# lgalke/aae-recommender

Measured on NVIDIA B200. Metric: AAE train item-sets/sec, higher is better.
Workload: dtype f32

## Files before the change

aae-recommender_b200/csrc/dec_out_tc.cu:

```cuda
#include "common.cuh"

#ifndef TC_WAIT_HINT
#define TC_WAIT_HINT 0x989680u
#endif
#ifndef TC_WAIT_SLEEP_NS
#define TC_WAIT_SLEEP_NS 40
#endif
#ifndef TC2_CW
#define TC2_CW 16
#endif
#ifndef TC2_G1_FIRST
#define TC2_G1_FIRST 1
#endif

namespace aae {
AAE_DEFINE_TRACE_SETTER(trace_set_tc)
namespace tc {

constexpr int TN = 32;
constexpr int BM = 128;
constexpr int NT = 512;
constexpr int CW = 8;
constexpr int CORE = 128;

__device__ __forceinline__ uint32_t smem_u32(const void* p) { return (uint32_t)__cvta_generic_to_shared(p); }

__device__ __forceinline__ uint64_t make_desc(uint32_t saddr, uint32_t lbo_bytes, uint32_t sbo_bytes) {
  uint64_t d = 0;
  d |= (uint64_t)((saddr >> 4) & 0x3FFFu);
  d |= (uint64_t)((lbo_bytes >> 4) & 0x3FFFu) << 16;
  d |= (uint64_t)((sbo_bytes >> 4) & 0x3FFFu) << 32;
  d |= (uint64_t)1 << 46;
  return d;
}
__device__ __forceinline__ uint64_t make_desc_sw(uint32_t saddr, uint32_t lbo_bytes, uint32_t sbo_bytes, uint32_t layout_type) {
  return make_desc(saddr, lbo_bytes, sbo_bytes) | ((uint64_t)layout_type << 61);
}
__host__ __device__ constexpr uint32_t make_idesc(int M, int N, int a_mn_major, int b_mn_major) {
  return (1u << 4) | (2u << 7) | (2u << 10) | ((uint32_t)a_mn_major << 15) | ((uint32_t)b_mn_major << 16) |
         ((uint32_t)(N >> 3) << 17) | ((uint32_t)(M >> 4) << 24);
}
__device__ __forceinline__ void mma_tf32(uint32_t d_tmem, uint64_t adesc, uint64_t bdesc, uint32_t idesc,
                                         uint32_t accumulate) {
  asm volatile(
      "{\n\t"
      ".reg .pred p;\n\t"
      "setp.ne.b32 p, %4, 0;\n\t"
      "tcgen05.mma.cta_group::1.kind::tf32 [%0], %1, %2, %3, p;\n\t"
      "}\n" ::"r"(d_tmem), "l"(adesc), "l"(bdesc), "r"(idesc), "r"(accumulate)
      : "memory");
}
__device__ __forceinline__ void mma_tf32_ts(uint32_t d_tmem, uint32_t a_tmem, uint64_t bdesc, uint32_t idesc,
                                            uint32_t accumulate) {
  asm volatile(
      "{\n\t"
      ".reg .pred p;\n\t"
      "setp.ne.b32 p, %4, 0;\n\t"
      "tcgen05.mma.cta_group::1.kind::tf32 [%0], [%1], %2, %3, p;\n\t"
      "}\n" ::"r"(d_tmem), "r"(a_tmem), "l"(bdesc), "r"(idesc), "r"(accumulate)
      : "memory");
}
__device__ __forceinline__ void mma_commit(uint64_t* bar) {
  asm volatile("tcgen05.commit.cta_group::1.mbarrier::arrive::one.shared::cluster.b64 [%0];" ::"r"(smem_u32(bar))
               : "memory");
}
__device__ __forceinline__ void mbar_init(uint64_t* bar, uint32_t count) {
  asm volatile("mbarrier.init.shared::cta.b64 [%0], %1;" ::"r"(smem_u32(bar)), "r"(count) : "memory");
}
__device__ __forceinline__ void mbar_wait(uint64_t* bar, uint32_t parity) {
  uint32_t done = 0;
  uint32_t spins = 0;
  while (!done) {
    if (spins) __nanosleep(TC_WAIT_SLEEP_NS);
    if (++spins > (1u << 22)) __trap();
    asm volatile(
        "{\n\t"
        ".reg .pred p;\n\t"
        "mbarrier.try_wait.parity.shared::cta.b64 p, [%1], %2, %3;\n\t"
        "selp.u32 %0, 1, 0, p;\n\t"
        "}\n"
        : "=r"(done)
        : "r"(smem_u32(bar)), "r"(parity), "r"(TC_WAIT_HINT)
        : "memory");
  }
}
__device__ __forceinline__ bool elect_one() {
  uint32_t pred;
  asm volatile(
      "{\n\t"
      ".reg .pred p;\n\t"
      "elect.sync _|p, 0xffffffff;\n\t"
      "selp.u32 %0, 1, 0, p;\n\t"
      "}\n"
      : "=r"(pred));
  return pred != 0;
}
__device__ __forceinline__ void fence_async_smem() { asm volatile("fence.proxy.async.shared::cta;" ::: "memory"); }
__device__ __forceinline__ void tc_fence_before() { asm volatile("tcgen05.fence::before_thread_sync;" ::: "memory"); }
__device__ __forceinline__ void tc_fence_after() { asm volatile("tcgen05.fence::after_thread_sync;" ::: "memory"); }

__device__ __forceinline__ void tmem_alloc(uint32_t* dst_smem, uint32_t ncols) {
  asm volatile("tcgen05.alloc.cta_group::1.sync.aligned.shared::cta.b32 [%0], %1;" ::"r"(smem_u32(dst_smem)),
               "r"(ncols)
               : "memory");
  asm volatile("tcgen05.relinquish_alloc_permit.cta_group::1.sync.aligned;" ::: "memory");
}
__device__ __forceinline__ void tmem_dealloc(uint32_t taddr, uint32_t ncols) {
  asm volatile("tcgen05.dealloc.cta_group::1.sync.aligned.b32 %0, %1;" ::"r"(taddr), "r"(ncols) : "memory");
}
__device__ __forceinline__ void tmem_ld16(uint32_t taddr, float* v) {
  uint32_t r[16];
  asm volatile(
      "tcgen05.ld.sync.aligned.32x32b.x16.b32 {%0,%1,%2,%3,%4,%5,%6,%7,%8,%9,%10,%11,%12,%13,%14,%15}, [%16];"
      : "=r"(r[0]), "=r"(r[1]), "=r"(r[2]), "=r"(r[3]), "=r"(r[4]), "=r"(r[5]), "=r"(r[6]), "=r"(r[7]), "=r"(r[8]),
        "=r"(r[9]), "=r"(r[10]), "=r"(r[11]), "=r"(r[12]), "=r"(r[13]), "=r"(r[14]), "=r"(r[15])
      : "r"(taddr)
      : "memory");
  asm volatile("tcgen05.wait::ld.sync.aligned;" ::: "memory");
#pragma unroll
  for (int i = 0; i < 16; ++i) v[i] = __uint_as_float(r[i]);
}

__device__ __forceinline__ void tmem_st16(uint32_t taddr, const float* v) {
  asm volatile(
      "tcgen05.st.sync.aligned.32x32b.x16.b32 [%0], {%1,%2,%3,%4,%5,%6,%7,%8,%9,%10,%11,%12,%13,%14,%15,%16};" ::"r"(taddr),
      "r"(__float_as_uint(v[0])), "r"(__float_as_uint(v[1])), "r"(__float_as_uint(v[2])), "r"(__float_as_uint(v[3])),
      "r"(__float_as_uint(v[4])), "r"(__float_as_uint(v[5])), "r"(__float_as_uint(v[6])), "r"(__float_as_uint(v[7])),
      "r"(__float_as_uint(v[8])), "r"(__float_as_uint(v[9])), "r"(__float_as_uint(v[10])), "r"(__float_as_uint(v[11])),
      "r"(__float_as_uint(v[12])), "r"(__float_as_uint(v[13])), "r"(__float_as_uint(v[14])), "r"(__float_as_uint(v[15]))
      : "memory");
}
__device__ __forceinline__ void tmem_st_wait() { asm volatile("tcgen05.wait::st.sync.aligned;" ::: "memory"); }

__device__ __forceinline__ void tmem_ld8(uint32_t taddr, float* v) {
  uint32_t r[8];
  asm volatile("tcgen05.ld.sync.aligned.32x32b.x8.b32 {%0,%1,%2,%3,%4,%5,%6,%7}, [%8];"
               : "=r"(r[0]), "=r"(r[1]), "=r"(r[2]), "=r"(r[3]), "=r"(r[4]), "=r"(r[5]), "=r"(r[6]), "=r"(r[7])
               : "r"(taddr)
               : "memory");
  asm volatile("tcgen05.wait::ld.sync.aligned;" ::: "memory");
#pragma unroll
  for (int i = 0; i < 8; ++i) v[i] = __uint_as_float(r[i]);
}
__device__ __forceinline__ void tmem_ld8_issue(uint32_t taddr, uint32_t* r) {
  asm volatile("tcgen05.ld.sync.aligned.32x32b.x8.b32 {%0,%1,%2,%3,%4,%5,%6,%7}, [%8];"
               : "=r"(r[0]), "=r"(r[1]), "=r"(r[2]), "=r"(r[3]), "=r"(r[4]), "=r"(r[5]), "=r"(r[6]), "=r"(r[7])
               : "r"(taddr)
               : "memory");
}
__device__ __forceinline__ void tmem_ld8_wait(uint32_t* r, float* v) {
  asm volatile("tcgen05.wait::ld.sync.aligned;"
               : "+r"(r[0]), "+r"(r[1]), "+r"(r[2]), "+r"(r[3]), "+r"(r[4]), "+r"(r[5]), "+r"(r[6]), "+r"(r[7])::"memory");
#pragma unroll
  for (int i = 0; i < 8; ++i) v[i] = __uint_as_float(r[i]);
}
__device__ __forceinline__ void tmem_st8(uint32_t taddr, const float* v) {
  asm volatile("tcgen05.st.sync.aligned.32x32b.x8.b32 [%0], {%1,%2,%3,%4,%5,%6,%7,%8};" ::"r"(taddr),
               "r"(__float_as_uint(v[0])), "r"(__float_as_uint(v[1])), "r"(__float_as_uint(v[2])),
               "r"(__float_as_uint(v[3])), "r"(__float_as_uint(v[4])), "r"(__float_as_uint(v[5])),
               "r"(__float_as_uint(v[6])), "r"(__float_as_uint(v[7]))
               : "memory");
}
template <int N> struct TmemIO;
template <> struct TmemIO<8> {
  static __device__ __forceinline__ void ld_issue(uint32_t taddr, uint32_t* r) {
    asm volatile("tcgen05.ld.sync.aligned.32x32b.x8.b32 {%0,%1,%2,%3,%4,%5,%6,%7}, [%8];"
                 : "=r"(r[0]), "=r"(r[1]), "=r"(r[2]), "=r"(r[3]), "=r"(r[4]), "=r"(r[5]), "=r"(r[6]), "=r"(r[7])
                 : "r"(taddr)
                 : "memory");
  }
  static __device__ __forceinline__ void ld_wait(uint32_t* r) {
    asm volatile("tcgen05.wait::ld.sync.aligned;"
                 : "+r"(r[0]), "+r"(r[1]), "+r"(r[2]), "+r"(r[3]), "+r"(r[4]), "+r"(r[5]), "+r"(r[6]), "+r"(r[7])::"memory");
  }
  static __device__ __forceinline__ void st(uint32_t taddr, const float* v) { tmem_st8(taddr, v); }
};
// ... 373 lines not shown
          if (k < H) {
            size_t off = (size_t)(v0 + v) * H + k;
            Wd3[off] = p; __stcs(mW + off, m); __stcs(vW + off, vv);
          } else {
            bd3[v0 + v] = p; mb[v0 + v] = m; vb[v0 + v] = vv;
          }
        }
      }
    }
    tc_fence_before();
    __syncthreads();
  }
  tc_fence_after();
  if (dh_started) {
    for (int c = cpart; c < g.Np / CW; c += NT / 128) {
      float d[CW];
      tmem_ld8(lane_addr + TM_DH + c * CW, d);
      if (brow < B) {
#pragma unroll
        for (int j = 0; j < CW; ++j) {
          int kk = c * CW + j;
          if (kk < H) atomicAdd(dh2 + (size_t)brow * H + kk, d[j]);
        }
      }
    }
  }
  float s = warp_sum(loss_local);
  if (lane == 0) red[warp] = s;
  tc_fence_before();
  __syncthreads();
  if (tid == 0) {
    double tot = 0.0;
    for (int w = 0; w < NT / 32; ++w) tot += (double)red[w];
    atomicAdd(loss_sum, tot);
  }
  if (warp == 0) tmem_dealloc(tmem, TMEM_COLS);
}

struct RowCursor2 {
  int pos, end, n0, n1, n2, n3;
};
__device__ __forceinline__ void cursor_init(RowCursor2& c, const int32_t* __restrict__ indices, int pos, int end) {
  c.pos = pos;
  c.end = end;
  c.n0 = (pos < end) ? __ldg(indices + pos) : 0x7fffffff;
  c.n1 = (pos + 1 < end) ? __ldg(indices + pos + 1) : 0x7fffffff;
  c.n2 = (pos + 2 < end) ? __ldg(indices + pos + 2) : 0x7fffffff;
  c.n3 = (pos + 3 < end) ? __ldg(indices + pos + 3) : 0x7fffffff;
}
__device__ __forceinline__ void cursor_advance(RowCursor2& c, const int32_t* __restrict__ indices) {
  c.n0 = c.n1;
  c.n1 = c.n2;
  c.n2 = c.n3;
  ++c.pos;
  c.n3 = (c.pos + 3 < c.end) ? __ldg(indices + c.pos + 3) : 0x7fffffff;
}
__device__ __forceinline__ uint32_t tile_targets2(RowCursor2& c, const int32_t* __restrict__ indices, int v0g) {
  while (c.n0 < v0g) cursor_advance(c, indices);
  uint32_t m = 0;
  while (c.n0 < v0g + TN) {
    m |= 1u << (c.n0 - v0g);
    cursor_advance(c, indices);
  }
  return m;
}
__device__ __forceinline__ void prefetch_l2_bulk(const void* p, uint32_t bytes) {
  if (bytes >= 16u)
    asm volatile("cp.async.bulk.prefetch.L2.global [%0], %1;" ::"l"(p), "r"(bytes & ~15u) : "memory");
}

constexpr uint32_t T2_Z = 0, T2_DW = 64, T2_DZH = 128, T2_DZL = 160, T2_DH = 192;

__device__ __forceinline__ void named_bar_sync(int id, int n) { asm volatile("bar.sync %0, %1;" ::"r"(id), "r"(n) : "memory"); }
__device__ __forceinline__ void named_bar_arrive(int id, int n) { asm volatile("bar.arrive %0, %1;" ::"r"(id), "r"(n) : "memory"); }

__device__ __forceinline__ float ex2_approx(float x) {
  float r;
  asm("ex2.approx.ftz.f32 %0, %1;" : "=f"(r) : "f"(x));
  return r;
}
__device__ __forceinline__ float lg2_approx(float x) {
  float r;
  asm("lg2.approx.ftz.f32 %0, %1;" : "=f"(r) : "f"(x));
  return r;
}
__device__ __forceinline__ float bce_neg_fast(float z, float inv_n, float& dz) {
  float u = ex2_approx(-1.4426950408889634f * fabsf(z));
  float t = 1.0f + u;
  float r = rcp_approx(t);
  float x = (z >= 0.f) ? r : u * r;
  dz = x * inv_n;
  return fmaf(lg2_approx(t), 0.6931471805599453f, fmaxf(z, 0.f));
}

template <int NCH, int NW>
__device__ __forceinline__ void make_wchunks_t(WChunk* wc, const Geom& g) {
  const int ncg = g.Kp / 4;
  const int r = threadIdx.x & 31, w = threadIdx.x >> 5;
#pragma unroll
  for (int j = 0; j < NCH; ++j) {
    int cg = w + NW * j;
    wc[j].goff = -2;
    if (cg < ncg) {
      int c = cg * 4;
      wc[j].goff = (c + 3 < g.H) ? r * g.H + c : (c == g.H ? -1 : -3);
    }
    wc[j].wb_off = (uint32_t)(r >> 3) * g.wb_sbo + (uint32_t)cg * CORE + (uint32_t)(r & 7) * 16u;
    wc[j].wt_off = (uint32_t)(cg >> 1) * g.wt_sbo + (uint32_t)(r >> 2) * g.wt_lbo + (uint32_t)(cg & 1) * 64u +
                   (uint32_t)(r & 3) * 4u;
  }
}
template <int NCH>
__device__ __forceinline__ void load_w_regs_t(float4* wr, const WChunk* wc, const float* __restrict__ Wd3,
                                              const float* __restrict__ bd3, int H, int v0, int nv) {
  const int r = threadIdx.x & 31;
#pragma unroll
  for (int j = 0; j < NCH; ++j) {
    float4 x = make_float4(0.f, 0.f, 0.f, 0.f);
    if (r < nv) {
      if (wc[j].goff >= 0) x = __ldcs(reinterpret_cast<const float4*>(Wd3 + (size_t)v0 * H + wc[j].goff));
      else if (wc[j].goff == -1) x.x = __ldg(bd3 + v0 + r);
    }
    wr[j] = x;
  }
}
template <int NCH>
__device__ __forceinline__ void store_wb_regs(const float4* wr, const WChunk* wc, unsigned char* wb_hi,
                                              unsigned char* wb_lo, bool with_lo) {
#pragma unroll
  for (int j = 0; j < NCH; ++j) {
    if (wc[j].goff == -2) continue;
    float4 x = wr[j];
    pin4(x);
    float4 h = make_float4(tf32_hi(x.x), tf32_hi(x.y), tf32_hi(x.z), tf32_hi(x.w));
    *reinterpret_cast<float4*>(wb_hi + wc[j].wb_off) = h;
    if (with_lo) *reinterpret_cast<float4*>(wb_lo + wc[j].wb_off) = make_float4(x.x - h.x, x.y - h.y, x.z - h.z, x.w - h.w);
  }
}
template <int NCH>
__device__ __forceinline__ void store_wt_regs(const float4* wr, const WChunk* wc, unsigned char* wt_hi,
                                              unsigned char* wt_lo, bool with_lo) {
#pragma unroll
  for (int j = 0; j < NCH; ++j) {
    if (wc[j].goff == -2) continue;
    float4 x = wr[j];
    float4 h = make_float4(tf32_hi(x.x), tf32_hi(x.y), tf32_hi(x.z), tf32_hi(x.w));
    float* th = reinterpret_cast<float*>(wt_hi + wc[j].wt_off);
    th[0] = h.x; th[4] = h.y; th[8] = h.z; th[12] = h.w;
    if (with_lo) {
      float* tl = reinterpret_cast<float*>(wt_lo + wc[j].wt_off);
      tl[0] = x.x - h.x; tl[4] = x.y - h.y; tl[8] = x.z - h.z; tl[12] = x.w - h.w;
    }
  }
}

__device__ __forceinline__ void mbar_arrive_expect_tx(uint64_t* bar, uint32_t bytes) {
  asm volatile("mbarrier.arrive.expect_tx.shared::cta.b64 _, [%0], %1;" ::"r"(smem_u32(bar)), "r"(bytes) : "memory");
}
__device__ __forceinline__ void mbar_arrive(uint64_t* bar) {
  asm volatile("mbarrier.arrive.shared::cta.b64 _, [%0];" ::"r"(smem_u32(bar)) : "memory");
}
__device__ __forceinline__ void bulk_g2s(void* dst_smem, const void* src, uint32_t bytes, uint64_t* bar) {
  asm volatile("cp.async.bulk.shared::cluster.global.mbarrier::complete_tx::bytes [%0], [%1], %2, [%3];" ::"r"(
                   smem_u32(dst_smem)),
               "l"(src), "r"(bytes), "r"(smem_u32(bar))
               : "memory");
}

#ifndef K3_PF_MV
#define K3_PF_MV 1
#endif
#ifndef K3_PF_AHEAD
#define K3_PF_AHEAD 4
#endif
#ifdef K3X_TRACE
static __device__ long long k3x_tr[32 * 16];
#define K3X_MARK(it, slot) do { if (blockIdx.x == 0 && (it) >= 8 && (it) < 40 && (threadIdx.x & 31) == 0) k3x_tr[((it) - 8) * 16 + (slot)] = clock64(); } while (0)
#else
#define K3X_MARK(it, slot) do { } while (0)
#endif
template <int CWT> struct Tc2Cfg {
  static constexpr int NPART = TN / CWT;
  static constexpr int NWE = 4 * NPART;
  static constexpr int NTT = 32 * NWE + 32;
  static constexpr int NTHR = 64 * NWE + 64;
  static constexpr int WCHT = 32 / NWE;
  static_assert(NTHR <= 1024, "two epilogue roles of 4*TN/CWT warps each: CWT = 16");
};
template <int SPLIT, int HC, int CWT, int MODE>
__global__ void __launch_bounds__(Tc2Cfg<CWT>::NTHR, 1) dec_out_train_tc2_kernel(
    const float* __restrict__ h2, int B, int Hrt, float* __restrict__ Wd3, float* __restrict__ bd3,
    float* __restrict__ mW, float* __restrict__ vW, float* __restrict__ mb, float* __restrict__ vb, int v_begin,
    int Vloc, const int32_t* __restrict__ indptr, const int32_t* __restrict__ indices, float inv_n,
    const aae_step_state* __restrict__ st, float* __restrict__ dh2, double* __restrict__ loss_sum, int smem_total,
    float* __restrict__ gW, float* __restrict__ gB) {
  constexpr bool kAdam = (MODE == 0 || MODE == 3);
  extern __shared__ __align__(1024) unsigned char smem[];
  __shared__ uint64_t bar_g1, bar_g23;
  __shared__ uint64_t bar_stage;
  __shared__ uint64_t bar_dw[2];
  __shared__ uint64_t bar_dwfree[2];
  __shared__ uint32_t tmem_base_s;
  constexpr int NPART = Tc2Cfg<CWT>::NPART, NWE = Tc2Cfg<CWT>::NWE, NTT = Tc2Cfg<CWT>::NTT, WCHT = Tc2Cfg<CWT>::WCHT;
  constexpr int NTHR = Tc2Cfg<CWT>::NTHR;
  __shared__ float red[NWE];
  const int H = HC ? HC : Hrt;
  const Geom g = make_geom(H);
  constexpr bool with_lo = (SPLIT == 3);
  const int BK = (B + 7) & ~7;
  const uint32_t hb_eff = (uint32_t)(BK / 8) * g.hb_sbo;
  unsigned char* hb_hi = smem;
  unsigned char* hb_lo = hb_hi + hb_eff;
  unsigned char* wb_hi = hb_lo + hb_eff;
  unsigned char* wb_lo = wb_hi + g.wb_bytes;
  unsigned char* wt_hi = wb_lo + g.wb_bytes;
  unsigned char* wt_lo = wt_hi + g.wt_bytes;
  unsigned char* dt_hi = wt_lo + g.wt_bytes;
  unsigned char* dt_lo = dt_hi + g.dt_bytes;
  float* sW = reinterpret_cast<float*>(dt_lo + g.dt_bytes);
  float* sM = sW + TN * H;
  float* sV = sM + TN * H;
  float* sB = sV + TN * H;
  const int tid = threadIdx.x, warp = tid >> 5, lane = tid & 31;
  const int n_tiles = (Vloc + TN - 1) / TN;
  const int G = gridDim.x;
  const int n_my = (n_tiles - (int)blockIdx.x + G - 1) / G;
  const uint32_t T2_HTH = T2_DH + (uint32_t)g.Np, T2_HTL = T2_HTH + (uint32_t)BK;

  trace_mark(TR_K3, 0);
  if (warp == 0) K3X_MARK(39, 0);
  if (warp == 2 * NWE) tmem_alloc(&tmem_base_s, TMEM_COLS);
  if (tid == 0) {
    mbar_init(&bar_g1, 1);
    mbar_init(&bar_g23, 1);
    mbar_init(&bar_stage, 1);
    mbar_init(&bar_dw[0], 1);
    mbar_init(&bar_dw[1], 1);
    mbar_init(&bar_dwfree[0], NWE);
    mbar_init(&bar_dwfree[1], NWE);
    asm volatile("fence.mbarrier_init.release.cluster;" ::: "memory");
  }
  constexpr int HB_BATCH = 5;
  const int ncg0 = g.Kp / 4;
  float4 hbx[HB_BATCH];
#pragma unroll
  for (int u = 0; u < HB_BATCH; ++u) {
    const int q = tid + u * NTHR;
    float4 x = make_float4(0.f, 0.f, 0.f, 0.f);
    if (q < BK * ncg0) {
      const int r = q / ncg0, c = (q - r * ncg0) * 4;
      if (r < B) {
        if (c + 3 < H) x = *reinterpret_cast<const float4*>(h2 + (size_t)r * H + c);
        else if (c == H) x.x = 1.0f;
      }
    }
    hbx[u] = x;
  }
  for (int q = tid; q < smem_total / 16; q += NTHR) reinterpret_cast<float4*>(smem)[q] = make_float4(0, 0, 0, 0);
  tc_fence_before();
  __syncthreads();
  tc_fence_after();
  const uint32_t tmem = tmem_base_s;
  if (warp == 0) K3X_MARK(39, 1);
  if (warp < 2 * NWE) {
    const int q4 = warp & 3, part = warp >> 2;
    const uint32_t lane_addr = tmem + ((uint32_t)(q4 * 32) << 16);
    const int k = q4 * 32 + lane;
    constexpr int NP4 = 2 * NPART;
    for (int c0 = part; c0 < BK / 8; c0 += 2 * NP4) {
      float x[16];
#pragma unroll
      for (int u = 0; u < 2; ++u) {
        const int c = c0 + u * NP4;
#pragma unroll
        for (int j = 0; j < 8; ++j) {
          const int b = c * 8 + j;
          float v = 0.f;
          if (c < BK / 8 && b < B) v = (k < H) ? h2[(size_t)b * H + k] : (k == H ? 1.0f : 0.f);
          x[u * 8 + j] = v;
        }
      }
#pragma unroll
      for (int u = 0; u < 2; ++u) {
        const int c = c0 + u * NP4;
        if (c < BK / 8) {
          float hi[8], lo[8];
#pragma unroll
          for (int j = 0; j < 8; ++j) {
            hi[j] = tf32_hi(x[u * 8 + j]);
            lo[j] = x[u * 8 + j] - hi[j];
          }
          tmem_st8(lane_addr + T2_HTH + c * 8, hi);
          if (with_lo) tmem_st8(lane_addr + T2_HTL + c * 8, lo);
        }
      }
    }
    tmem_st_wait();
  }
#pragma unroll
  for (int u = 0; u < HB_BATCH; ++u) {
    const int q = tid + u * NTHR;
    if (q < BK * ncg0) {
      const int r = q / ncg0, cg = q - r * ncg0;
      store_split4(hb_hi, hb_lo, r, cg, g.hb_sbo, hbx[u], with_lo);
    }
  }
// ... 338 lines not shown
    if (warp == 0) K3X_MARK(39, 6);
    {
      const int nch = g.Np / CWT;
      const int rot = (int)(blockIdx.x % (unsigned)nch);
      for (int c = cpart; c < nch; c += NPART) {
        int cc = c + rot;
        if (cc >= nch) cc -= nch;
        float d[CWT];
        {
          uint32_t dr[CWT];
          TmemIO<CWT>::ld_issue(lane_addr + T2_DH + cc * CWT, dr);
          TmemIO<CWT>::ld_wait(dr);
#pragma unroll
          for (int j = 0; j < CWT; ++j) d[j] = __uint_as_float(dr[j]);
        }
        if (brow < B) {
          float* dst = dh2 + (size_t)brow * H + cc * CWT;
#pragma unroll
          for (int j = 0; j < CWT; j += 4) {
            if (cc * CWT + j + 3 < H)
              asm volatile("red.global.add.v4.f32 [%0], {%1, %2, %3, %4};" ::"l"(dst + j), "f"(d[j]), "f"(d[j + 1]),
                           "f"(d[j + 2]), "f"(d[j + 3])
                           : "memory");
          }
        }
      }
    }
    float s = warp_sum(loss_local);
    if (lane == 0) red[warp] = s;
    if (warp == 0) K3X_MARK(39, 7);
  } else {
    const int we = warp - NWE;
    const int q4 = we & 3, cpart = we >> 2;
    const uint32_t lane_addr = tmem + ((uint32_t)(q4 * 32) << 16);
    const int brow = q4 * 32 + lane;
    const AdamK ak = adam_load(st, 0);
    const int kb = H & 31;
    const bool bias_warp = (q4 == (H >> 5));
    const int jb = brow - (H + 1);
    const bool is_bias = (jb >= 0 && jb < CWT);
    float* const eW = is_bias ? bd3 : Wd3;
    float* const eM = is_bias ? mb : mW;
    float* const eV = is_bias ? vb : vW;
    const float* const sWp = is_bias ? sB + cpart * CWT + jb : sW + cpart * CWT * H + brow;
    const float* const sMp = is_bias ? sB + TN + cpart * CWT + jb : sM + cpart * CWT * H + brow;
    const float* const sVp = is_bias ? sB + 2 * TN + cpart * CWT + jb : sV + cpart * CWT * H + brow;
    const int ecnt_full = is_bias ? 1 : (brow < H ? CWT : 0);
    uint32_t phase_e = 0, ph_dw0 = 0, ph_dw1 = 0;
    const uint32_t rt_zero = (uint32_t)smem_total >> 31;
    for (int jt = 0; jt < n_my; ++jt) {
      const int tile = blockIdx.x + jt * G;
      const int v0 = tile * TN;
      const int nv = min(TN, Vloc - v0);
      size_t eoff;
      int ecnt;
      if (is_bias) {
        eoff = (size_t)v0 + cpart * CWT + jb;
        ecnt = (cpart * CWT + jb < nv) ? 1 : 0;
      } else {
        eoff = (size_t)(v0 + cpart * CWT) * H + brow;
        ecnt = (brow < H) ? max(0, min(CWT, nv - cpart * CWT)) : 0;
      }
      float* pW = eW + eoff;
      float* pM = eM + eoff;
      float* pV = eV + eoff;
      float* pG = (MODE != 0) ? ((is_bias ? gB : gW) + eoff) : nullptr;
      float pw[CWT], pm[CWT], pv[CWT], pg[CWT];
#pragma unroll
      for (int j = 0; j < CWT; ++j) pw[j] = pm[j] = pv[j] = 0.f;
      if (MODE == 2 || MODE == 3) {
#pragma unroll
        for (int j = 0; j < CWT; ++j) pg[j] = (j < ecnt) ? pG[(size_t)j * H] : 0.f;
      }
      if (warp == NWE) K3X_MARK(jt, 8);
      mbar_wait(&bar_stage, phase_e);
      phase_e ^= 1;
      if (warp == NWE) K3X_MARK(jt, 9);
#ifdef K3X_NO_E2LD
      if (false) {
#else
      if (kAdam) {
#endif
        if (nv == TN) {
#pragma unroll
          for (int j = 0; j < CWT; ++j) {
            if (j < ecnt_full) {
              pw[j] = sWp[j * H];
              pm[j] = sMp[j * H];
              pv[j] = sVp[j * H];
            }
          }
        } else {
#pragma unroll
          for (int j = 0; j < CWT; ++j) {
            if (j < ecnt) {
              pw[j] = pW[(size_t)j * H];
              pm[j] = pM[(size_t)j * H];
              pv[j] = pV[(size_t)j * H];
            }
          }
        }
      }
      if (jt + 1 < n_my) {
        uint32_t dep = 0u;
#pragma unroll
        for (int j = 0; j < CWT; ++j) dep ^= __float_as_uint(pw[j]) ^ __float_as_uint(pm[j]) ^ __float_as_uint(pv[j]);
        named_bar_arrive(2 + (int)(dep & rt_zero), NTT);
      }
      if (jt & 1) { mbar_wait(&bar_dw[1], ph_dw1); ph_dw1 ^= 1; } else { mbar_wait(&bar_dw[0], ph_dw0); ph_dw0 ^= 1; }
      tc_fence_after();
      if (warp == NWE) K3X_MARK(jt, 10);
      float gw[CWT];
      {
        uint32_t gr[CWT];
        TmemIO<CWT>::ld_issue(lane_addr + T2_DW + (uint32_t)(jt & 1) * 32u + cpart * CWT, gr);
        TmemIO<CWT>::ld_wait(gr);
#pragma unroll
        for (int j = 0; j < CWT; ++j) gw[j] = __uint_as_float(gr[j]);
      }
      tc_fence_before();
      __syncwarp();
      if (lane == 0) mbar_arrive(&bar_dwfree[jt & 1]);
      if (bias_warp) {
        float gb = 0.f;
#pragma unroll
        for (int j = 0; j < CWT; ++j) {
          float t = __shfl_sync(0xffffffffu, gw[j], kb);
          if (jb == j) gb = t;
        }
        if (is_bias) gw[0] = gb;
      }
      if (MODE == 2 || MODE == 3) {
#pragma unroll
        for (int j = 0; j < CWT; ++j) gw[j] += pg[j];
      }
      if (kAdam) {
        float dn[CWT];
#ifndef K3X_NO_E2MATH
#pragma unroll
        for (int j = 0; j < CWT; ++j) pm[j] = fmaf(ak.w1, gw[j] - pm[j], pm[j]);
#pragma unroll
        for (int j = 0; j < CWT; ++j) pv[j] = fmaf(ak.w2 * gw[j], gw[j], pv[j] * ak.beta2);
#pragma unroll
        for (int j = 0; j < CWT; ++j) dn[j] = fmaf(sqrt_approx(pv[j]), ak.inv_bc2_sqrt, ak.eps);
#pragma unroll
        for (int j = 0; j < CWT; ++j) dn[j] = pm[j] * rcp_approx(dn[j]);
#pragma unroll
        for (int j = 0; j < CWT; ++j) pw[j] = fmaf(-ak.step_size, dn[j], pw[j]);
#else
#pragma unroll
        for (int j = 0; j < CWT; ++j) { dn[j] = gw[j]; pw[j] += dn[j]; }
#endif
#ifndef K3X_NO_E2ST
#pragma unroll
        for (int j = 0; j < CWT; ++j) {
          if (j < ecnt) {
            pW[(size_t)j * H] = pw[j];
            __stcs(pM + (size_t)j * H, pm[j]);
            __stcs(pV + (size_t)j * H, pv[j]);
          }
        }
#else
        if (pw[0] + pm[1] + pv[2] == 1.2345e30f) pW[0] = pw[3];
#endif
      } else {
#pragma unroll
        for (int j = 0; j < CWT; ++j)
          if (j < ecnt) pG[(size_t)j * H] = gw[j];
      }
      if (warp == NWE) K3X_MARK(jt, 7);
    }
  }
  tc_fence_before();
  __syncthreads();
  if (tid == 0) {
    double tot = 0.0;
    for (int w = 0; w < NWE; ++w) tot += (double)red[w];
    atomicAdd(loss_sum, tot);
  }
  if (warp == 0) K3X_MARK(39, 8);
  if (warp == 2 * NWE) tmem_dealloc(tmem, TMEM_COLS);
  trace_mark(TR_K3, 1);
}

template <int SPLIT>
__global__ void __launch_bounds__(NT, 1) dec_out_scores_tc_kernel(const float* __restrict__ h2, int B, int H,
                                                                  const float* __restrict__ Wd3,
                                                                  const float* __restrict__ bd3, int Vloc,
                                                                  int apply_sigmoid, float* __restrict__ out,
                                                                  int64_t ldo) {
  constexpr int split = SPLIT;
  extern __shared__ __align__(1024) unsigned char smem[];
  __shared__ uint64_t bar_mma;
  __shared__ uint32_t tmem_base_s;
  const Geom g = make_geom(H);
  unsigned char* hb_hi = smem;
  unsigned char* hb_lo = hb_hi + g.hb_bytes;
  unsigned char* wb_hi = hb_lo + g.hb_bytes;
  unsigned char* wb_lo = wb_hi + g.wb_bytes;
  const bool with_lo = (split == 3);
  const int tid = threadIdx.x, warp = tid >> 5, lane = tid & 31;
  const int q4 = warp & 3, cpart = warp >> 2;
  const int n_tiles = (Vloc + TN - 1) / TN;
  const int n_chunks = (B + BM - 1) / BM;
  if (warp == 0) tmem_alloc(&tmem_base_s, 32);
  if (tid == 0) {
    mbar_init(&bar_mma, 1);
    asm volatile("fence.mbarrier_init.release.cluster;" ::: "memory");
  }
  tc_fence_before();
  __syncthreads();
  tc_fence_after();
  const uint32_t tmem = tmem_base_s;
  const uint32_t lane_addr = tmem + ((uint32_t)(q4 * 32) << 16);
  uint32_t phase = 0;
  const uint32_t idesc_g1 = make_idesc(BM, TN, 0, 0);
  const SmemOp op_hb = make_op(hb_hi, hb_lo, CORE, g.hb_sbo, 2 * CORE);
  const SmemOp op_wb = make_op(wb_hi, wb_lo, CORE, g.wb_sbo, 2 * CORE);
  WChunk wc[WCH];
  make_wchunks(wc, g);
  for (int chunk = blockIdx.y; chunk < n_chunks; chunk += gridDim.y) {
    const int b0 = chunk * BM, nb = min(BM, B - b0);
    __syncthreads();
    fill_hb(hb_hi, hb_lo, g, h2, b0, nb, with_lo);
    for (int tile = blockIdx.x; tile < n_tiles; tile += gridDim.x) {
      const int v0 = tile * TN, nv = min(TN, Vloc - v0);
      float4 wr[WCH];
      load_w_regs(wr, wc, Wd3, bd3, H, v0, nv);
      store_w_regs(wr, wc, wb_hi, wb_lo, nullptr, nullptr, with_lo);
      fence_async_smem();
      __syncthreads();
      if (warp == 0) {
        tc_fence_after();
        if (elect_one()) {
          issue_gemm<SPLIT>(tmem, op_hb, op_wb, g.Kp / 8, idesc_g1, 0u);
          mma_commit(&bar_mma);
        }
        __syncwarp();
      }
      mbar_wait(&bar_mma, phase);
      phase ^= 1;
      tc_fence_after();
      float z[CW];
      tmem_ld8(lane_addr + cpart * CW, z);
      const int brow = q4 * 32 + lane;
      if (brow < nb) {
        float* orow = out + (size_t)(b0 + brow) * ldo + v0 + cpart * CW;
#pragma unroll
        for (int j = 0; j < CW; ++j) {
          if (cpart * CW + j < nv) {
            float s = z[j];
            if (apply_sigmoid) s = 1.0f / (1.0f + expf(-s));
            orow[j] = s;
          }
        }
      }
      tc_fence_before();
      __syncthreads();
    }
  }
  if (warp == 0) tmem_dealloc(tmem, 32);
}

__global__ void __launch_bounds__(NT, 1) tc_selftest_kernel(int mode_in, const float* __restrict__ A,
                                                            const float* __restrict__ Bm, float* __restrict__ D,
                                                            int split) {
  extern __shared__ __align__(1024) unsigned char smem[];
  __shared__ uint64_t bar_mma;
  __shared__ uint32_t tmem_base_s;
  const Geom g = make_geom(100);
  int mode = mode_in;
  unsigned char* hb_hi = smem;
  unsigned char* hb_lo = hb_hi + g.hb_bytes;
  unsigned char* wb_hi = hb_lo + g.hb_bytes;
  unsigned char* wb_lo = wb_hi + g.wb_bytes;
  unsigned char* wt_hi = wb_lo + g.wb_bytes;
  unsigned char* wt_lo = wt_hi + g.wt_bytes;
  unsigned char* dt_hi = wt_lo + g.wt_bytes;
  unsigned char* dt_lo = dt_hi + g.dt_bytes;
  const bool with_lo = (split == 3);
  const int tid = threadIdx.x, warp = tid >> 5, lane = tid & 31;
  const int q4 = warp & 3, cpart = warp >> 2;
  if (warp == 0) tmem_alloc(&tmem_base_s, TMEM_COLS);
  if (tid == 0) {
    mbar_init(&bar_mma, 1);
    asm volatile("fence.mbarrier_init.release.cluster;" ::: "memory");
  }
  for (int q = tid; q < (int)(smem_bytes(g) - 256) / 16; q += NT) reinterpret_cast<float4*>(smem)[q] = make_float4(0, 0, 0, 0);
  tc_fence_before();
  __syncthreads();
  tc_fence_after();
  const uint32_t tmem = tmem_base_s;
  const uint32_t lane_addr = tmem + ((uint32_t)(q4 * 32) << 16);
  const int row = q4 * 32 + lane;
  auto split_store = [&](unsigned char* hi, unsigned char* lo, int r, int c, uint32_t lbo, uint32_t sbo, float x) {
    uint32_t off = (uint32_t)(r >> 3) * sbo + (uint32_t)(c >> 2) * lbo + (uint32_t)(r & 7) * 16u + (uint32_t)(c & 3) * 4u;
    float h = tf32_hi(x);
    *reinterpret_cast<float*>(hi + off) = h;
    if (with_lo) *reinterpret_cast<float*>(lo + off) = x - h;
  };
  const int variant = mode >> 4;
  mode &= 15;
  unsigned char* pb_hi = smem;
  unsigned char* pb_lo = smem + 16384;
  if (mode == 6 || mode == 7) {
    const int acols = (mode == 6) ? TN : BM;
    const uint32_t th = (mode == 6) ? TM_DZH : TM_HTH, tl = (mode == 6) ? TM_DZL : TM_HTL;
    for (int c = cpart; c < acols / CW; c += NT / 128) {
      float hi[CW], lo[CW];
#pragma unroll
      for (int j = 0; j < CW; ++j) {
        float x = A[(size_t)row * acols + c * CW + j];
        hi[j] = tf32_hi(x);
        lo[j] = x - hi[j];
      }
      tmem_st8(lane_addr + th + c * CW, hi);
      if (with_lo) tmem_st8(lane_addr + tl + c * CW, lo);
    }
    tmem_st_wait();
    const int nN = (mode == 6) ? g.Np : TN, nK = (mode == 6) ? TN : BM;
    for (int q = tid; q < nN * nK; q += NT) {
      const int n = q / nK, kk = q % nK;
      const int blk = n >> 5, nn = n & 31;
      const int sw = (variant == 2) ? 0 : (kk & 3);
      const uint32_t off = (uint32_t)blk * 4096u + (uint32_t)kk * 128u + (uint32_t)(((nn >> 3) ^ sw) * 32) + (uint32_t)(nn & 7) * 4u;
      const float x = Bm[q], h = tf32_hi(x);
      *reinterpret_cast<float*>(pb_hi + off) = h;
      if (with_lo) *reinterpret_cast<float*>(pb_lo + off) = x - h;
    }
  } else if (mode == 1) {
    for (int q = tid; q < BM * g.Kp; q += NT) split_store(hb_hi, hb_lo, q / g.Kp, q % g.Kp, CORE, g.hb_sbo, A[q]);
    for (int q = tid; q < TN * g.Kp; q += NT) split_store(wb_hi, wb_lo, q / g.Kp, q % g.Kp, CORE, g.wb_sbo, Bm[q]);
  } else {
    const int acols = (mode == 2) ? TN : BM;
    const uint32_t th = (mode == 2) ? TM_DZH : TM_HTH, tl = (mode == 2) ? TM_DZL : TM_HTL;
    for (int c = cpart; c < acols / CW; c += NT / 128) {
      float hi[CW], lo[CW];
#pragma unroll
      for (int j = 0; j < CW; ++j) {
        float x = A[(size_t)row * acols + c * CW + j];
        hi[j] = tf32_hi(x);
        lo[j] = x - hi[j];
      }
      tmem_st8(lane_addr + th + c * CW, hi);
      if (with_lo) tmem_st8(lane_addr + tl + c * CW, lo);
    }
    tmem_st_wait();
    if (mode == 2)
      for (int q = tid; q < g.Np * TN; q += NT) split_store(wt_hi, wt_lo, q / TN, q % TN, g.wt_lbo, g.wt_sbo, Bm[q]);
    else
      for (int q = tid; q < TN * BM; q += NT) split_store(dt_hi, dt_lo, q / BM, q % BM, g.dt_lbo, g.dt_sbo, Bm[q]);
  }
  fence_async_smem();
  tc_fence_before();
  __syncthreads();
  if (warp == 0) {
    tc_fence_after();
    const SmemOp o_hb = make_op(hb_hi, hb_lo, CORE, g.hb_sbo, 2 * CORE), o_wb = make_op(wb_hi, wb_lo, CORE, g.wb_sbo, 2 * CORE);
    const SmemOp o_wt = make_op(wt_hi, wt_lo, g.wt_lbo, g.wt_sbo, 2 * g.wt_lbo);
    const SmemOp o_dt = make_op(dt_hi, dt_lo, g.dt_lbo, g.dt_sbo, 2 * g.dt_lbo);
    const bool leader = elect_one();
    if (leader && (mode == 6 || mode == 7)) {
      uint32_t lbo = 4096u, sbo = 512u;
      if (variant == 1) { lbo = 512u; sbo = 4096u; }
      if (variant == 3) sbo = 1024u;
      SmemOp o;
      o.hi = make_desc_sw(smem_u32(pb_hi), lbo, sbo, 1u);
      o.lo = make_desc_sw(smem_u32(pb_lo), lbo, sbo, 1u);
      o.step16 = 1024u >> 4;
      if (mode == 6) {
        if (split == 3) issue_gemm_ts<3>(tmem + TM_DH, tmem + TM_DZH, tmem + TM_DZL, o, TN / 8, make_idesc(BM, g.Np, 0, 1), 0u);
        else issue_gemm_ts<1>(tmem + TM_DH, tmem + TM_DZH, tmem + TM_DZL, o, TN / 8, make_idesc(BM, g.Np, 0, 1), 0u);
      } else {
        if (split == 3) issue_gemm_ts<3>(tmem + TM_DW, tmem + TM_HTH, tmem + TM_HTL, o, BM / 8, make_idesc(BM, TN, 0, 1), 0u);
        else issue_gemm_ts<1>(tmem + TM_DW, tmem + TM_HTH, tmem + TM_HTL, o, BM / 8, make_idesc(BM, TN, 0, 1), 0u);
      }
      mma_commit(&bar_mma);
    } else if (leader) {
      if (split == 3) {
        if (mode == 1) issue_gemm<3>(tmem + TM_Z, o_hb, o_wb, g.Kp / 8, make_idesc(BM, TN, 0, 0), 0u);
        else if (mode == 2) issue_gemm_ts<3>(tmem + TM_DH, tmem + TM_DZH, tmem + TM_DZL, o_wt, TN / 8, make_idesc(BM, g.Np, 0, 0), 0u);
        else issue_gemm_ts<3>(tmem + TM_DW, tmem + TM_HTH, tmem + TM_HTL, o_dt, BM / 8, make_idesc(BM, TN, 0, 0), 0u);
      } else {
        if (mode == 1) issue_gemm<1>(tmem + TM_Z, o_hb, o_wb, g.Kp / 8, make_idesc(BM, TN, 0, 0), 0u);
        else if (mode == 2) issue_gemm_ts<1>(tmem + TM_DH, tmem + TM_DZH, tmem + TM_DZL, o_wt, TN / 8, make_idesc(BM, g.Np, 0, 0), 0u);
        else issue_gemm_ts<1>(tmem + TM_DW, tmem + TM_HTH, tmem + TM_HTL, o_dt, BM / 8, make_idesc(BM, TN, 0, 0), 0u);
      }
      mma_commit(&bar_mma);
    }
    __syncwarp();
  }
  mbar_wait(&bar_mma, 0);
  tc_fence_after();
  const int ncols = (mode == 2 || mode == 6) ? g.Np : TN;
  const uint32_t tsrc = (mode == 1) ? TM_Z : ((mode == 2 || mode == 6) ? TM_DH : TM_DW);
  for (int c = cpart; c < ncols / CW; c += NT / 128) {
    float d[CW];
    tmem_ld8(lane_addr + tsrc + c * CW, d);
#pragma unroll
    for (int j = 0; j < CW; ++j) D[(size_t)row * ncols + c * CW + j] = d[j];
  }
  tc_fence_before();
  __syncthreads();
  if (warp == 0) tmem_dealloc(tmem, TMEM_COLS);
}

constexpr int PN = 128;
constexpr int P_NWE = 16;
constexpr int P_NT = 32 * P_NWE + 32;
constexpr int P_CW = PN / 4;
constexpr int P_WCH = 7;
constexpr uint32_t P_T_AHI = 256, P_T_ALO = 384, P_TMEM_COLS = 512;

struct SelArgs {
  const float* h2; int B, H;
  const float* Wd3; const float* bd3; int Vloc, v_begin;
  int tile_stride, n_sel;
  int filter;
  float* out; long long ldo; int out_by_visit, apply_sigmoid;
  const float* tau; int tau_stride; int32_t* cnt; float* cand_val; int32_t* cand_idx; int cap_sub;
};

struct PChunks {
  int goff[P_WCH];
  uint32_t soff[P_WCH];
};
__device__ __forceinline__ void p_load_w(float4* wr, const PChunks& pc, const float* __restrict__ wtile,
                                         const float* __restrict__ btile, bool rv) {
#pragma unroll
  for (int j = 0; j < P_WCH; ++j) {
    float4 x = make_float4(0.f, 0.f, 0.f, 0.f);
    if (rv) {
      if (pc.goff[j] >= 0) x = __ldg(reinterpret_cast<const float4*>(wtile + pc.goff[j]));
      else if (pc.goff[j] == -1) x.x = __ldg(btile);
    }
    wr[j] = x;
  }
}
__device__ __forceinline__ void p_store_w(const float4* wr, const PChunks& pc, unsigned char* hi, unsigned char* lo,
                                          bool with_lo) {
#pragma unroll
  for (int j = 0; j < P_WCH; ++j) {
    if (pc.goff[j] == -2) continue;
    const float4 x = wr[j];
    const float4 h = make_float4(tf32_hi(x.x), tf32_hi(x.y), tf32_hi(x.z), tf32_hi(x.w));
    *reinterpret_cast<float4*>(hi + pc.soff[j]) = h;
    if (with_lo) *reinterpret_cast<float4*>(lo + pc.soff[j]) = make_float4(x.x - h.x, x.y - h.y, x.z - h.z, x.w - h.w);
  }
}

template <int SPLIT>
__global__ void __launch_bounds__(P_NT, 1) dec_out_select_kernel(SelArgs a) {
  extern __shared__ __align__(1024) unsigned char smem[];
  __shared__ uint64_t bar_mma[2], bar_ready[2];
  __shared__ uint32_t tmem_base_s;
  constexpr bool with_lo = (SPLIT == 3);
  const Geom g = make_geom(a.H);
  const uint32_t wb_bytes = (PN / 8) * g.wb_sbo;
  unsigned char* wst = smem;
  const int tid = threadIdx.x, warp = tid >> 5, lane = tid & 31;
  const int ncg = g.Kp / 4;
  const int n_chunks = (a.B + BM - 1) / BM;
  const int n_my = ((int)blockIdx.x < a.n_sel) ? (a.n_sel - (int)blockIdx.x + (int)gridDim.x - 1) / (int)gridDim.x : 0;
  for (uint32_t q = tid; q < 4u * wb_bytes / 16u; q += P_NT) reinterpret_cast<float4*>(wst)[q] = make_float4(0.f, 0.f, 0.f, 0.f);
  if (warp == P_NWE) tmem_alloc(&tmem_base_s, P_TMEM_COLS);
  if (tid == 0) {
    mbar_init(&bar_mma[0], 1);
    mbar_init(&bar_mma[1], 1);
    mbar_init(&bar_ready[0], P_NWE);
    mbar_init(&bar_ready[1], P_NWE);
    asm volatile("fence.mbarrier_init.release.cluster;" ::: "memory");
  }
  tc_fence_before();
  __syncthreads();
  tc_fence_after();
  const uint32_t tmem = tmem_base_s;
  const uint32_t idesc = make_idesc(BM, PN, 0, 0);
  uint32_t ph0 = 0, ph1 = 0;
  for (int chunk = blockIdx.y; chunk < n_chunks; chunk += gridDim.y) {
    const int b0 = chunk * BM, nb = min(BM, a.B - b0);
    __syncthreads();
    if (warp < P_NWE) {
      const int q4 = warp & 3, cpart = warp >> 2;
      const uint32_t lane_addr = tmem + ((uint32_t)(q4 * 32) << 16);
      const int brow = q4 * 32 + lane;
      for (int c = cpart; c < g.Kp / 8; c += 4) {
        float hi[8], lo[8];
#pragma unroll
        for (int j = 0; j < 8; ++j) {
          const int kk = c * 8 + j;
          float x = 0.f;
          if (brow < nb) x = (kk < a.H) ? __ldg(a.h2 + (size_t)(b0 + brow) * a.H + kk) : (kk == a.H ? 1.0f : 0.f);
          hi[j] = tf32_hi(x);
          lo[j] = x - hi[j];
        }
        tmem_st8(lane_addr + P_T_AHI + c * 8, hi);
        if (with_lo) tmem_st8(lane_addr + P_T_ALO + c * 8, lo);
      }
      tmem_st_wait();
    }
    tc_fence_before();
    __syncthreads();
    tc_fence_after();
    if (warp == P_NWE) {
      const SmemOp op_w0 = make_op(wst, wst + wb_bytes, CORE, g.wb_sbo, 2 * CORE);
      const SmemOp op_w1 = make_op(wst + 2 * wb_bytes, wst + 3 * wb_bytes, CORE, g.wb_sbo, 2 * CORE);
      for (int it = 0; it < n_my; ++it) {
        const int s = it & 1;
        mbar_wait(&bar_ready[s], s ? ph1 : ph0);
        if (s) ph1 ^= 1; else ph0 ^= 1;
        tc_fence_after();
        if (elect_one()) {
          issue_gemm_ts<SPLIT>(tmem + (uint32_t)(s * PN), tmem + P_T_AHI, tmem + P_T_ALO, s ? op_w1 : op_w0, g.Kp / 8,
                               idesc, 0u);
          mma_commit(&bar_mma[s]);
        }
        __syncwarp();
      }
    } else {
      const int q4 = warp & 3, cpart = warp >> 2;
      const uint32_t lane_addr = tmem + ((uint32_t)(q4 * 32) << 16);
      const int brow = q4 * 32 + lane;
      const bool rowv = brow < nb;
      float tau = __int_as_float(0x7f800000);
      if (a.filter && rowv) tau = a.tau[(size_t)(b0 + brow) * a.tau_stride];
      const int nsub = (int)gridDim.x * 4, sub = (int)blockIdx.x * 4 + cpart;
      const size_t sub_base = ((size_t)(b0 + brow) * nsub + sub) * (size_t)a.cap_sub;
      int my_cnt = 0;
      const int lrow = warp * 8 + (lane & 7);
      PChunks pc;
#pragma unroll
      for (int j = 0; j < P_WCH; ++j) {
        const int cg = (lane >> 3) + 4 * j, c = cg * 4;
        pc.goff[j] = (cg < ncg) ? ((c + 3 < a.H) ? lrow * a.H + c : (c == a.H ? -1 : -3)) : -2;
        pc.soff[j] = (uint32_t)(lrow >> 3) * g.wb_sbo + (uint32_t)cg * CORE + (uint32_t)(lrow & 7) * 16u;
      }
      const int tile_step = (int)gridDim.x * a.tile_stride * PN;
      const int v_first = (int)blockIdx.x * a.tile_stride * PN;
      auto load_tile = [&](float4* wr, int v0) {
        p_load_w(wr, pc, a.Wd3 + (size_t)v0 * a.H, a.bd3 + v0 + lrow, v0 + lrow < a.Vloc);
      };
      float4 wr[P_WCH];
      for (int p = 0; p < 2 && p < n_my; ++p) {
        load_tile(wr, v_first + p * tile_step);
        p_store_w(wr, pc, wst + 2 * p * wb_bytes, wst + (2 * p + 1) * wb_bytes, with_lo);
        fence_async_smem();
        __syncwarp();
        if (lane == 0) mbar_arrive(&bar_ready[p]);
// ... 259 lines not shown
```

Measured before the change: 65940.

## Vectorize Adam weight/moment stores via quad shuffle transpose; add test GEMM modes

In the fused decoder-output Adam epilogue, each quad of lanes transposes its per-column values with warp shuffles so W, m and v can be written as float4 stores along H instead of scalar strided stores. This aims to cut store instruction count and improve coalescing for full tiles. A scalar fallback remains for partial tiles. The change also adds new test-harness GEMM modes (8-10) with N=112, which look like validation or probe paths rather than training speed work.

```diff
diff --git a/aae-recommender_b200/csrc/dec_out_tc.cu b/aae-recommender_b200/csrc/dec_out_tc.cu
--- a/aae-recommender_b200/csrc/dec_out_tc.cu
+++ b/aae-recommender_b200/csrc/dec_out_tc.cu
@@ -22,6 +22,7 @@
 constexpr int NT = 512;
 constexpr int CW = 8;
 constexpr int CORE = 128;
+constexpr int IM_N = 112;
 
 __device__ __forceinline__ uint32_t smem_u32(const void* p) { return (uint32_t)__cvta_generic_to_shared(p); }
 
@@ -701,6 +702,18 @@
       tl[0] = x.x - h.x; tl[4] = x.y - h.y; tl[8] = x.z - h.z; tl[12] = x.w - h.w;
     }
   }
+}
+
+__device__ __forceinline__ float sel4(const float* a, int i) {
+  return i == 0 ? a[0] : (i == 1 ? a[1] : (i == 2 ? a[2] : a[3]));
+}
+__device__ __forceinline__ float4 xpose4(const float* a, int s) {
+  const float r0 = sel4(a, s);
+  const float r1 = __shfl_xor_sync(0xffffffffu, sel4(a, s ^ 1), 1);
+  const float r2 = __shfl_xor_sync(0xffffffffu, sel4(a, s ^ 2), 2);
+  const float r3 = __shfl_xor_sync(0xffffffffu, sel4(a, s ^ 3), 3);
+  const float rr[4] = {r0, r1, r2, r3};
+  return make_float4(sel4(rr, s), sel4(rr, s ^ 1), sel4(rr, s ^ 2), sel4(rr, s ^ 3));
 }
 
 __device__ __forceinline__ void mbar_arrive_expect_tx(uint64_t* bar, uint32_t bytes) {
@@ -1345,12 +1358,29 @@
         for (int j = 0; j < CWT; ++j) { dn[j] = gw[j]; pw[j] += dn[j]; }
 #endif
 #ifndef K3X_NO_E2ST
-#pragma unroll
-        for (int j = 0; j < CWT; ++j) {
-          if (j < ecnt) {
-            pW[(size_t)j * H] = pw[j];
-            __stcs(pM + (size_t)j * H, pm[j]);
-            __stcs(pV + (size_t)j * H, pv[j]);
+        const bool st4 = (nv == TN) && (brow < H);
+        if (nv == TN) {
+          const int s = lane & 3;
+          const size_t o4 = (size_t)(v0 + cpart * CWT + s) * H + (brow & ~3);
+#pragma unroll
+          for (int j0 = 0; j0 < CWT; j0 += 4) {
+            const float4 w4 = xpose4(pw + j0, s), m4 = xpose4(pm + j0, s), v4 = xpose4(pv + j0, s);
+            if (st4) {
+              const size_t o = o4 + (size_t)j0 * H;
+              *reinterpret_cast<float4*>(Wd3 + o) = w4;
+              __stcs(reinterpret_cast<float4*>(mW + o), m4);
+              __stcs(reinterpret_cast<float4*>(vW + o), v4);
+            }
+          }
+        }
+        if (!st4) {
+#pragma unroll
+          for (int j = 0; j < CWT; ++j) {
+            if (j < ecnt) {
+              pW[(size_t)j * H] = pw[j];
+              __stcs(pM + (size_t)j * H, pm[j]);
+              __stcs(pV + (size_t)j * H, pv[j]);
+            }
           }
         }
 #else
@@ -1524,6 +1554,40 @@
   } else if (mode == 1) {
     for (int q = tid; q < BM * g.Kp; q += NT) split_store(hb_hi, hb_lo, q / g.Kp, q % g.Kp, CORE, g.hb_sbo, A[q]);
     for (int q = tid; q < TN * g.Kp; q += NT) split_store(wb_hi, wb_lo, q / g.Kp, q % g.Kp, CORE, g.wb_sbo, Bm[q]);
+  } else if (mode == 8 || mode == 10) {
+    const int ka = (mode == 8) ? g.Kp : TN;
+    const uint32_t sbo = (uint32_t)(ka / 4) * CORE;
+    unsigned char* a_hi = smem;
+    unsigned char* a_lo = a_hi + (BM / 8) * sbo;
+    unsigned char* b_hi = a_lo + (BM / 8) * sbo;
+    unsigned char* b_lo = b_hi + (IM_N / 8) * sbo;
+    for (int q = tid; q < BM * ka; q += NT) {
+      const int r = q / ka, c = q % ka;
+      if (mode == 8) {
+        const uint32_t off = core_off(r, c, sbo);
+        const float x = A[q];
+        *reinterpret_cast<float*>(a_hi + off) = x;
+        if (with_lo) *reinterpret_cast<float*>(a_lo + off) = x - tf32_hi(x);
+      } else {
+        split_store(a_hi, a_lo, r, c, CORE, sbo, A[q]);
+      }
+    }
+    for (int q = tid; q < IM_N * ka; q += NT) split_store(b_hi, b_lo, q / ka, q % ka, CORE, sbo, Bm[q]);
+  } else if (mode == 9) {
+    for (int c = cpart; c < g.Kp / CW; c += NT / 128) {
+      float hi[CW], lo[CW];
+#pragma unroll
+      for (int j = 0; j < CW; ++j) {
+        float x = A[(size_t)row * g.Kp + c * CW + j];
+        hi[j] = tf32_hi(x);
+        lo[j] = x - hi[j];
+      }
+      tmem_st8(lane_addr + TM_HTH + c * CW, hi);
+      if (with_lo) tmem_st8(lane_addr + TM_HTL + c * CW, lo);
+    }
+    tmem_st_wait();
+    const uint32_t sbo = (uint32_t)(g.Kp / 4) * CORE;
+    for (int q = tid; q < IM_N * g.Kp; q += NT) split_store(smem, smem + (IM_N / 8) * sbo, q / g.Kp, q % g.Kp, CORE, sbo, Bm[q]);
   } else {
     const int acols = (mode == 2) ? TN : BM;
     const uint32_t th = (mode == 2) ? TM_DZH : TM_HTH, tl = (mode == 2) ? TM_DZL : TM_HTL;
@@ -1569,6 +1633,21 @@
         else issue_gemm_ts<1>(tmem + TM_DW, tmem + TM_HTH, tmem + TM_HTL, o, BM / 8, make_idesc(BM, TN, 0, 1), 0u);
       }
       mma_commit(&bar_mma);
+    } else if (leader && mode >= 8) {
+      const uint32_t idesc = make_idesc(BM, IM_N, 0, 0);
+      const int ka = (mode == 10) ? TN : g.Kp;
+      const uint32_t sbo = (uint32_t)(ka / 4) * CORE;
+      if (mode == 9) {
+        const SmemOp ob = make_op(smem, smem + (IM_N / 8) * sbo, CORE, sbo, 2 * CORE);
+        if (split == 3) issue_gemm_ts<3>(tmem + TM_DH, tmem + TM_HTH, tmem + TM_HTL, ob, ka / 8, idesc, 0u);
+        else issue_gemm_ts<1>(tmem + TM_DH, tmem + TM_HTH, tmem + TM_HTL, ob, ka / 8, idesc, 0u);
+      } else {
+        const SmemOp oa = make_op(smem, smem + (BM / 8) * sbo, CORE, sbo, 2 * CORE);
+        const SmemOp ob = make_op(smem + 2 * (BM / 8) * sbo, smem + (2 * (BM / 8) + IM_N / 8) * sbo, CORE, sbo, 2 * CORE);
+        if (split == 3) issue_gemm<3>(tmem + TM_DH, oa, ob, ka / 8, idesc, 0u);
+        else issue_gemm<1>(tmem + TM_DH, oa, ob, ka / 8, idesc, 0u);
+      }
+      mma_commit(&bar_mma);
     } else if (leader) {
       if (split == 3) {
         if (mode == 1) issue_gemm<3>(tmem + TM_Z, o_hb, o_wb, g.Kp / 8, make_idesc(BM, TN, 0, 0), 0u);
@@ -1585,8 +1664,8 @@
   }
   mbar_wait(&bar_mma, 0);
   tc_fence_after();
-  const int ncols = (mode == 2 || mode == 6) ? g.Np : TN;
-  const uint32_t tsrc = (mode == 1) ? TM_Z : ((mode == 2 || mode == 6) ? TM_DH : TM_DW);
+  const int ncols = (mode == 2 || mode == 6) ? g.Np : (mode >= 8 ? IM_N : TN);
+  const uint32_t tsrc = (mode == 1) ? TM_Z : ((mode == 2 || mode == 6 || mode >= 8) ? TM_DH : TM_DW);
   for (int c = cpart; c < ncols / CW; c += NT / 128) {
     float d[CW];
     tmem_ld8(lane_addr + tsrc + c * CW, d);
```

Result: slower. 23340, median of 6 (-64.6%).
